# wing02/MyLdpcCppApi

Hardware: AMD Instinct MI355X
Metric: decoded Mbit/s (info bits), DVB-S2 N=64800 rate-1/2, 50 iters (higher is better)
Workload: dtype f32; 1 GPU; DVB-S2-profile (64800,32400) rate-1/2 (seeded IRA table with the standard's structure, E=226799), batch 4096 frames per GPU, 50 iterations, sum-product fp32 (probability domain), all-zero codeword + AWGN sigma=0.95 (no frame converges), early termination on, inputs resident in HBM; global_batch=4096, frames_per_gpu=4096, algo=sp, frames_per_launch=4096, parallelism=frames sharded over 1 GPU(s), all-gather of decoded bytes, frames_converged=0

## Files before the change

### myldpccppapi_amd/capi.py

```python
import ctypes

import numpy as np

from . import _lib
from ._lib import DecoderConfig, DecodeStats, LdpcError

ALGO_SP, ALGO_MS, ALGO_LAYERED, ALGO_MS_FUSED, ALGO_LAYERED_HOST = 0, 1, 2, 3, 4
MSG_F32, MSG_F16 = 0, 1
PACK_BYTES, PACK_BITS = 0, 1
CODE_PACKED, CODE_BITS = 0, 1
CODE_FORMATS = {"packed": CODE_PACKED, "bits": CODE_BITS}
PARITY_KINDS = {1: "dual_diagonal", 2: "staircase"}
HOST_INPUT = {"auto": 0, "staged": 1, "lock_pages": 2}
ALGOS = {"sp": ALGO_SP, "ms": ALGO_MS, "layered": ALGO_LAYERED, "ms_fused": ALGO_MS_FUSED,
         "layered_host": ALGO_LAYERED_HOST}

TUNE_FIELDS = {"fused": 0, "ldsp": 2, "ldsp_ext": 4, "ldsp_pack": 6, "link_narrow": 8, "check_wide": 10,
               "syn_xcd": 12, "fused_pack": 14, "fused_loop": 16, "device_tail": 18, "merge": 20, "link_deep": 22, "link_half": 24,
               "link_guided": 26, "tiles_first": 28}
TUNE_INTS = ("rows_per_wave", "cols_per_wave", "link_rows", "compact", "ldsp_grid", "ldsp_per_cu", "ldsp_waves", "place", "q_order")


def apply_tune(cfg, tune):
    flags, shape = 0, 0
    for k, v in (tune or {}).items():
        if k in TUNE_FIELDS:
            if v is not None:
                flags |= (1 if v else 2) << TUNE_FIELDS[k]
        elif k == "ldsp_per_cu":
            shape |= int(v) & 255
        elif k == "ldsp_waves":
            shape |= (int(v) & 255) << 8
        elif k in TUNE_INTS:
            setattr(cfg, "tune_" + k, int(v))
        else:
            raise KeyError("unknown tuning field %r" % k)
    cfg.tune_flags, cfg.tune_ldsp_shape = flags, shape


def hbm_probe(device=0, nbytes=1 << 30, reps=5, by_policy=False):
    g = ctypes.c_double(0.0)
    two = (ctypes.c_double * 2)(0.0, 0.0)
    _lib.check(_lib.load().ldpc_hbm_probe_device(int(device), int(nbytes), int(reps), ctypes.byref(g), two))
    return (g.value, two[0], two[1]) if by_policy else g.value


def hbm_sustained(device=0, nbytes=1 << 30, milliseconds=300):
    g = ctypes.c_double(0.0)
    _lib.check(_lib.load().ldpc_hbm_sustained_device(int(device), int(nbytes), int(milliseconds), ctypes.byref(g)))
    return g.value


def tune_from_env(env=None):
    import os
    env = os.environ if env is None else env
    t = {}
    for name, key in (("FUSED", "fused"), ("LDSP", "ldsp"), ("LDSP_EXT", "ldsp_ext"), ("LDSP_PACK", "ldsp_pack"),
                      ("LINK_NARROW", "link_narrow"), ("CHECK_WIDE", "check_wide"), ("SYN_XCD", "syn_xcd"),
                      ("FUSED_LOOP", "fused_loop"), ("DEVICE_TAIL", "device_tail"), ("MERGE", "merge"), ("LINK_DEEP", "link_deep"), ("LINK_HALF", "link_half"),
                      ("LINK_GUIDED", "link_guided"), ("TILES_FIRST", "tiles_first")):
        if "LDPC_TUNE_" + name in env:
            t[key] = int(env["LDPC_TUNE_" + name]) != 0
    if "LDPC_TUNE_NO_PACK" in env:
        t["fused_pack"] = False
    for name, key in (("RPW", "rows_per_wave"), ("CPW", "cols_per_wave"), ("LDSP_GRID", "ldsp_grid"),
                      ("LDSP_PER_CU", "ldsp_per_cu"), ("LDSP_WAVES", "ldsp_waves")):
        if "LDPC_TUNE_" + name in env:
            t[key] = int(env["LDPC_TUNE_" + name])
    for name, key in (("LINK_RPW", "link_rows"), ("COMPACT", "compact")):
# ... 275 lines not shown
```

### myldpccppapi_amd/csrc/flood_kernels.hpp

```cpp
#pragma once

#include <hip/hip_runtime.h>
#include <stdint.h>

#include "ldpc_expf.h"

namespace ldpc {

constexpr int kAlgoSP = 0;
constexpr int kAlgoMS = 1;
constexpr int kAlgoMSC = 2;
constexpr int kCompactCapacity = 512;
constexpr int kLastCapacity = 64;
constexpr int kBlock = 256;
constexpr int kWavesPerBlock = 4;
constexpr int kMaxUnrolledDegree = 16;
constexpr int kMaxUnrolledCheckDegreeMS = 32;

#ifndef LDPC_NT_LOAD
#define LDPC_NT_LOAD 1
#endif
#ifndef LDPC_NT_STORE
#define LDPC_NT_STORE 1
#endif
// ... 508 lines not shown
    const int32_t *__restrict__ extra_deg;
    int32_t n_extra;
    int32_t link_blocks;
    int32_t n_big, small_rows;
};

__host__ __device__ inline void link_chunk_rows(int c, int rows_per_wave, int n_big, int small_rows, int n_rows,
                                               int *rb, int *re)
{
    int b, e;
    if (c < n_big) { b = c * rows_per_wave; e = b + rows_per_wave; }
    else { b = n_big * rows_per_wave + (c - n_big) * small_rows; e = b + small_rows; }
    *rb = b < n_rows ? b : n_rows;
    *re = e < n_rows ? e : n_rows;
}
__host__ __device__ inline int link_chunk_count(int rows_per_wave, int n_big, int small_rows, int n_rows)
{
    const int rest = n_rows - n_big * rows_per_wave;
    return n_big + (rest > 0 ? (rest + small_rows - 1) / small_rows : 0);
}

template <int ALGO, int V, typename T>
__device__ __forceinline__ void link_extra_rows(const CheckArgs &a, const LinkArgs &g, int tile, int block)
{
    constexpr size_t F = 64 * V;
    const int lane = threadIdx.x & 63;
    const int w = (block - g.link_blocks) * kWavesPerBlock + wave_id_in_block();
    if (w >= g.n_extra) return;
    const T *Qu = static_cast<const T *>(a.Q) + (size_t)tile * (size_t)a.E * F;
    T *Rt = static_cast<T *>(a.R) + (size_t)tile * (size_t)a.E * F + (size_t)lane * V;
    check_row_generic<ALGO, V, T>(Qu, (unsigned)lane * V, Rt, g.extra_e0[w], g.extra_deg[w], a.qpos, ms_corr_of(a));
}

#ifdef LDPC_LINK_WIDE_WAVES
#define LDPC_LINK_WIDE_ATTR __attribute__((amdgpu_waves_per_eu(LDPC_LINK_WIDE_WAVES, LDPC_LINK_WIDE_WAVES)))
#else
#define LDPC_LINK_WIDE_ATTR
#endif
template <int ALGO, int D, int V, typename T>
__global__ __launch_bounds__(kBlock) LDPC_LINK_WIDE_ATTR void check_link_kernel(const CheckArgs a, const LinkArgs g)
{
    constexpr size_t F = 64 * V;
    const int lane = threadIdx.x & 63;
    const GridPos gp = grid_pos(a.tiles_first);
    const int tile = tile_select<V>(a.tail, a.done, gp.row);
    if (tile < 0) return;
    if (gp.block >= g.link_blocks) { link_extra_rows<ALGO, V, T>(a, g, tile, gp.block); return; }
    const int wave = gp.block * kWavesPerBlock + wave_id_in_block();
    int r_begin, r_end;
    link_chunk_rows(wave, a.rows_per_wave, g.n_big, g.small_rows, a.n_rows, &r_begin, &r_end);
    const size_t lane_off = (size_t)lane * V;
    const unsigned lane_q = (unsigned)lane * V;
    const T *Qt = static_cast<const T *>(a.Q) + (size_t)tile * (size_t)a.E * F;
    T *Qwt = static_cast<T *>(g.Qw) + (size_t)tile * (size_t)a.E * F;
    T *Rt = static_cast<T *>(a.R) + (size_t)tile * (size_t)a.E * F + lane_off;
    const T *chan_t = static_cast<const T *>(g.chan) + (size_t)tile * (size_t)g.N * F + lane_off;
    uint64_t *hard_t = g.hard + (size_t)tile * (size_t)g.N * V;
    uint64_t frozen[V];
#pragma unroll
    for (int v = 0; v < V; ++v) frozen[v] = a.done[(size_t)tile * V + v];

    int pend_col = -1, pend_edge = 0, pend_kb = 0;
    float pend_r[V];
#pragma unroll
    for (int v = 0; v < V; ++v) pend_r[v] = 0.0f;

    float x[D][V];
    int qc[D], qn[D];
#pragma unroll
    for (int k = 0; k < D; ++k) qc[k] = qn[k] = 0;
    if (r_begin < r_end) {
        row_slots<D>(a.qpos, a.cls_e0[r_begin], lane, qc);
#pragma unroll
        for (int k = 0; k < D; ++k) vload<V>(x[k], Qt + (size_t)qc[k] * F + lane_q);
    }
    for (int r = r_begin; r < r_end; ++r) {
        const int e0 = a.cls_e0[r];
        const int next_col = (r + 1 < r_end) ? g.link_col[r] : -1;
        const int pos = g.link_pos[r];
        const int ka = next_col >= 0 ? (pos & 255) : -1;
        const int kb = pend_col >= 0 ? pend_kb : -1;
        if (r + 1 < r_end) row_slots<D>(a.qpos, a.cls_e0[r + 1], lane, qn);
        float ch[V];
        uint64_t old_w[V];
        if (pend_col >= 0) {
            vload<V>(ch, chan_t + (size_t)pend_col * F);
#pragma unroll
            for (int v = 0; v < V; ++v) old_w[v] = hard_t[(size_t)pend_col * V + v];
        }
        float out[D][V];
        if (ALGO == kAlgoSP) check_sp<D, V>(x, out); else if (ALGO == kAlgoMS) check_ms<D, V>(x, out); else check_ms<D, V, true, T>(x, out, ms_corr_of(a));
        if (r + 1 < r_end) {
#pragma unroll
            for (int k = 0; k < D; ++k) vload<V>(x[k], Qt + (size_t)qn[k] * F + lane_q);
        }
#pragma unroll
        for (int k = 0; k < D; ++k)
            if ((k != ka && k != kb) || g.store_all) vstore<V>(Rt + (size_t)(e0 + k) * F, out[k]);

        if (pend_col >= 0) {
            float rr[2][V], q[2][V];
#pragma unroll
            for (int v = 0; v < V; ++v) {
                rr[0][v] = pend_r[v];
                float t = out[0][v];
#pragma unroll
                for (int k = 1; k < D; ++k) t = (k == kb) ? out[k][v] : t;
                rr[1][v] = t;
            }
            uint64_t new_w[V];
            if (ALGO == kAlgoSP) {
                float f0[V], f1[V];
                var_sp<2, V>(ch, rr, q, f0, f1);
#pragma unroll
                for (int v = 0; v < V; ++v) {
                    const bool oldb = (old_w[v] >> lane) & 1ull;
                    const bool b = (f0[v] > f1[v]) ? false : ((f0[v] < f1[v]) ? true : oldb);
                    new_w[v] = __ballot(b);
                }
            } else {
#pragma unroll
                for (int v = 0; v < V; ++v) {
                    float p = ch[v];
                    p += rr[0][v];
                    p += rr[1][v];
                    q[0][v] = p - rr[0][v];
                    q[1][v] = p - rr[1][v];
                    new_w[v] = __ballot(!(p > 0.0f));
                }
            }
            if (lane == 0) {
#pragma unroll
                for (int v = 0; v < V; ++v)
                    hard_t[(size_t)pend_col * V + v] = (old_w[v] & frozen[v]) | (new_w[v] & ~frozen[v]);
            }
            if (g.write_q) {
                int qw1 = qc[0];
#pragma unroll
                for (int k = 1; k < D; ++k) qw1 = (k == kb) ? qc[k] : qw1;
                vstore<V>(Qwt + (size_t)pend_edge * F + lane_q, q[0]);
                vstore<V>(Qwt + (size_t)qw1 * F + lane_q, q[1]);
            }
        }
        pend_col = next_col;
        if (next_col >= 0) {
            pend_edge = qc[0];
#pragma unroll
            for (int k = 1; k < D; ++k) pend_edge = (k == ka) ? qc[k] : pend_edge;
            pend_kb = (pos >> 8) & 255;
#pragma unroll
            for (int v = 0; v < V; ++v) {
                float t = out[0][v];
#pragma unroll
                for (int k = 1; k < D; ++k) t = (k == ka) ? out[k][v] : t;
                pend_r[v] = t;
            }
        }
#pragma unroll
        for (int k = 0; k < D; ++k) qc[k] = qn[k];
    }
}

template <int V> __device__ __forceinline__ uint64_t compress_stride(uint64_t x)
{
    if (V == 1) return x;
    if (V == 2) {
        x &= 0x5555555555555555ull;
        x = (x | (x >> 1)) & 0x3333333333333333ull;
        x = (x | (x >> 2)) & 0x0f0f0f0f0f0f0f0full;
        x = (x | (x >> 4)) & 0x00ff00ff00ff00ffull;
        x = (x | (x >> 8)) & 0x0000ffff0000ffffull;
        x = (x | (x >> 16)) & 0x00000000ffffffffull;
        return x;
    }
    x &= 0x1111111111111111ull;
    x = (x | (x >> 3)) & 0x0303030303030303ull;
    x = (x | (x >> 6)) & 0x000f000f000f000full;
    x = (x | (x >> 12)) & 0x000000ff000000ffull;
    x = (x | (x >> 24)) & 0x000000000000ffffull;
    return x;
}

template <int ALGO, int D, int V, typename T, int W = 1>
__global__ __launch_bounds__(kBlock) void check_link_narrow_kernel(const CheckArgs a, const LinkArgs g)
{
    constexpr size_t F = 64 * V;
    constexpr int SUBS = V / W;
    constexpr int FB = 64 / SUBS;
    const int lane = threadIdx.x & 63;
    const GridPos gp = grid_pos(a.tiles_first);
    const int tile = tile_select<V>(a.tail, a.done, gp.row);
    if (tile < 0) return;
// ... 1053 lines not shown
```

### myldpccppapi_amd/csrc/ldpc_hip.hip

```cpp
#include <hip/hip_runtime.h>

#include <algorithm>
#include <chrono>
#include <cstdarg>
#include <cstdio>
#include <cstdlib>
#include <cstring>
#include <map>
#include <memory>
#include <new>
#include <string>
#include <thread>
#include <vector>

#include "../../include/ldpc_hip.h"
#include "flood_kernels.hpp"
#include "flood_tables.hpp"
#include "layered_kernels.hpp"
#include "fused_kernels.hpp"
#include "ldsp_kernels.hpp"
#include "engines.hpp"
#include "channel_kernels.hpp"
#include "tune.hpp"
#include "host_stage.hpp"
// ... 138 lines not shown
    DevBuf<int32_t> row_ptr, edge_col, col_ptr, col_edge;
    DevBuf<int32_t> qpos, col_qedge;
    std::vector<int32_t> h_qpos;
    DevBuf<uint8_t> chan, Q, R;
    int msg_size = 4;
    InitFn init_fn = nullptr;
    DevBuf<uint64_t> hard, failw, done;
    DevBuf<int32_t> iters, active;
    std::vector<RowClass> row_classes;
    std::vector<ColClass> col_classes;
    std::vector<ClassGroup> check_groups, var_groups;
    std::vector<int> check_solo, var_solo;
    CheckGroupFn check_group_fn[kCheckBuckets] = {};
    int check_group_width = 1;
    VarGroupFn var_group_fn[kVarBuckets] = {};
    DevBuf<int32_t> extra_e0, extra_deg;
    int n_extra = 0;
    int64_t extra_edges = 0;
    CheckFn check_fn[ldpc::kMaxUnrolledCheckDegreeMS + 1] = {};
    CheckFn check_fn_wide[ldpc::kMaxUnrolledCheckDegreeMS + 1] = {};
    int max_check_unrolled = ldpc::kMaxUnrolledDegree;
    LinkFn link_fn[ldpc::kMaxUnrolledDegree + 1] = {};
    LinkFn link_narrow_fn[ldpc::kMaxUnrolledDegree + 1] = {};
    LinkFn link_deep_fn[ldpc::kMaxUnrolledDegree + 1] = {};
    LinkFn link_half_fn[ldpc::kMaxUnrolledDegree + 1] = {};
    int tune_link_deep = 0;
    ldpc::Tune tune;
    int tune_link_narrow = 1;
    bool link_calibrated = false;
    float link_cal_ms[3] = {0, 0, 0};
    int place_candidates = 0, place_kept = 0;
    float place_ms[16] = {};
    int link_rpw = 16;
    int tune_link_guided = 0;
    int tune_tiles_first = 0;
    int cus = 256;
    VarFn var_fn[ldpc::kMaxUnrolledDegree + 1] = {};

    ldpc::LayeredPlan layered;
    ldpc::FusedPlan fused;
    bool use_fused = false;
    ldpc::LdspPlan ldsp;
    bool use_ldsp = false;
    bool ms_corr = false;
    float ms_scale = 1.0f, ms_offset = 0.0f;

    hipStream_t stream = nullptr, copy_stream = nullptr;
    struct HostSlot {
        DevBuf<float> llr;
        DevBuf<uint8_t> out;
        DevBuf<int32_t> iters;
        uint8_t *h_out = nullptr;
        int32_t *h_iters = nullptr;
        uint8_t *h_head = nullptr;
        hipEvent_t h2d_done = nullptr, all_done = nullptr;
        bool busy = false;
        int64_t off = 0, n = 0, dst = 0, copy_bytes = 0;
        int32_t *h_sum = nullptr;
        int g_iterations = 0, g_tiles = 0, g_children = 0, g_child_f[3] = {0, 0, 0};
    } slot[3];
    struct CallCounts { bool valid = false; int32_t iterations = 0, batch_time = 0; int64_t frames = 0, converged = 0, frame_rounds = 0; } call;
    bool suppress_poll = false;
    int32_t *h_active = nullptr;
    struct RingChunk { uint8_t *h = nullptr; hipEvent_t ev = nullptr; bool used = false; };
    std::vector<RingChunk> ring;
    size_t ring_next = 0;
// ... 407 lines not shown
        }
    }
    d->last_iterations = launched;
    d->last_tiles = tiles;
    if (resume) return LDPC_OK;

    HIP_TRY(span_begin(d, s, 3));
    if (use_tail) tail_scatter_kernel<V><<<2048, kBlock, 0, s>>>(ta);
    {
        PackArgs pa{d->hard.p, out_dev, d->iters.p, iters_dev, frames, out_bytes, d->N, d->cfg.K,
                    d->cfg.pack_mode};
        if (d->cfg.pack_mode == LDPC_PACK_BYTES) {
            if (out_dev && frames) pack_kernel<V><<<pack_grid<V>(d->cfg.K, tiles), kBlock, 0, s>>>(pa);
        } else {
            const int64_t n = std::max<int64_t>(out_bytes, frames);
            dim3 grid((unsigned)((n + kBlock - 1) / kBlock));
            if (out_dev && frames) pack_kernel<V><<<grid, kBlock, 0, s>>>(pa);
        }
        summary_kernel<V><<<(unsigned)((frames + 255) / 256), 256, 0, s>>>(
            d->iters.p, d->done.p, d->failw.p, frames, 1, d->summary.p);
        if (!d->is_child && d->cfg.poll_interval == 0 && freeze && !d->summary_pending) {
            HIP_TRY(hipMemcpyAsync(d->h_summary, d->summary.p, 2 * sizeof(int32_t), hipMemcpyDeviceToHost, s));
            HIP_TRY(hipEventRecord(d->ev_summary, s));
            d->summary_pending = true;
        }
    }
    HIP_TRY(span_end(d, s));
    HIP_TRY(hipGetLastError());
    return LDPC_OK;
}

int build_classes(ldpc_decoder *d, const ldpc_graph *g)
{
    std::map<int, std::vector<int32_t>> rows_by_deg, cols_by_deg, rowids_by_deg;
    for (int32_t m = 0; m < g->M; ++m) {
        const int deg = g->row_ptr[m + 1] - g->row_ptr[m];
        if (deg > 0) { rows_by_deg[deg].push_back(g->row_ptr[m]); rowids_by_deg[deg].push_back(m); }
    }
    std::vector<char> fused_col((size_t)g->N, 0);
    d->row_classes.resize(rows_by_deg.size());
    size_t i = 0;
    for (auto &kv : rows_by_deg) {
        RowClass &rc = d->row_classes[i++];
        rc.degree = kv.first;
        rc.count = (int)kv.second.size();
        rc.h_e0 = kv.second;
        HIP_TRY(rc.e0.upload(kv.second));
        const std::vector<int32_t> &ids = rowids_by_deg[kv.first];
        const int rpw = d->link_rpw;
        if (rpw >= 2 && rc.degree >= 2 && rc.degree <= ldpc::kMaxUnrolledDegree) {
            rc.n_big = (rc.count + rpw - 1) / rpw;
            rc.small_rows = rpw;
            const int small = std::max(2, rpw / 4);
            const bool forced = ldpc::tune_forced_on(d->tune_link_guided);
            if ((d->T >= 4 || forced) && small < rpw && !ldpc::tune_forced_off(d->tune_link_guided)) {
                const int64_t last_generation = (int64_t)d->cus * 16 / d->T;
                int64_t big = (int64_t)rc.n_big - last_generation;
                if (big <= 0 && forced) big = rc.n_big - std::max(1, rc.n_big / 3);
                if (big > 0) { rc.n_big = (int)big; rc.small_rows = small; }
            }
            std::vector<char> chunk_end((size_t)rc.count, 0);
            for (int c = 0, nc = ldpc::link_chunk_count(rpw, rc.n_big, rc.small_rows, rc.count); c < nc; ++c) {
                int rb, re;
                ldpc::link_chunk_rows(c, rpw, rc.n_big, rc.small_rows, rc.count, &rb, &re);
                if (re > rb) chunk_end[(size_t)re - 1] = 1;
            }
            std::vector<int32_t> lcol((size_t)rc.count, -1), lpos((size_t)rc.count, 0);
            for (int idx = 0; idx + 1 < rc.count; ++idx) {
                if (chunk_end[idx]) continue;
                const int32_t m = ids[idx], m2 = ids[idx + 1];
                for (int32_t p = g->row_ptr[m]; p < g->row_ptr[m + 1]; ++p) {
                    const int32_t c = g->cols[p];
                    if (g->col_ptr[c + 1] - g->col_ptr[c] != 2 || fused_col[c]) continue;
                    const int32_t ea = g->col_edge[g->col_ptr[c]], eb = g->col_edge[g->col_ptr[c] + 1];
                    if (ea != p || g->rows[eb] != m2) continue;
                    lcol[idx] = c;
                    lpos[idx] = (p - g->row_ptr[m]) | ((eb - g->row_ptr[m2]) << 8);
                    fused_col[c] = 1;
                    ++rc.linked;
                    break;
                }
            }
            if (rc.linked * 4 >= rc.count) {
                HIP_TRY(rc.link_col.upload(lcol));
                HIP_TRY(rc.link_pos.upload(lpos));
            } else {
                for (int idx = 0; idx < rc.count; ++idx)
                    if (lcol[idx] >= 0) fused_col[lcol[idx]] = 0;
                rc.linked = 0;
            }
        }
    }
    for (int32_t n = 0; n < g->N; ++n) {
        const int deg = g->col_ptr[n + 1] - g->col_ptr[n];
        if (!fused_col[n]) cols_by_deg[deg].push_back(n);
    }
    d->col_classes.resize(cols_by_deg.size());
    i = 0;
    for (auto &kv : cols_by_deg) {
        ColClass &cc = d->col_classes[i++];
        cc.degree = kv.first;
        cc.count = (int)kv.second.size();
        std::vector<int32_t> edges;
        edges.reserve((size_t)cc.count * std::max(cc.degree, 1));
        for (int32_t n : kv.second)
            for (int32_t p = g->col_ptr[n]; p < g->col_ptr[n + 1]; ++p) edges.push_back(g->col_edge[p]);
        if (edges.empty()) edges.push_back(0);
        HIP_TRY(cc.col.upload(kv.second));
        HIP_TRY(cc.edge.upload(edges));
    }
    {
        d->h_qpos.assign((size_t)g->E, -1);
        int64_t slot = 0;
        if (d->tune.q_order >= 0)
            for (ColClass &cc : d->col_classes) {
                cc.q_base = slot;
                const std::vector<int32_t> &members = cols_by_deg[cc.degree];
                for (size_t ci = 0; ci < members.size(); ++ci)
                    for (int k = 0; k < cc.degree; ++k)
                        d->h_qpos[(size_t)g->col_edge[(size_t)g->col_ptr[members[ci]] + k]] = (int32_t)(slot + (int64_t)k * cc.count + (int64_t)ci);
                slot += (int64_t)cc.degree * cc.count;
            }
        for (int64_t e = 0; e < g->E; ++e)
            if (d->h_qpos[(size_t)e] < 0) d->h_qpos[(size_t)e] = d->tune.q_order >= 0 ? (int32_t)slot++ : (int32_t)e;
        std::vector<int32_t> cq((size_t)g->E);
        for (int64_t p = 0; p < g->E; ++p) cq[(size_t)p] = d->h_qpos[(size_t)g->col_edge[(size_t)p]];
        HIP_TRY(d->qpos.upload(d->h_qpos));
        HIP_TRY(d->col_qedge.upload(cq));
    }
    return LDPC_OK;
}

int plan_launches(ldpc_decoder *d)
{
    using ldpc::GroupClass;
    const int V = d->V;
    const bool merge = ldpc::tune_pick(d->tune.merge, true) && !d->tune_check_wide;
    d->check_groups.clear(); d->var_groups.clear(); d->check_solo.clear(); d->var_solo.clear();
    d->n_extra = 0; d->extra_edges = 0;
    int linked_classes = 0;
    int64_t unlinked_rows = 0;
    for (auto &rc : d->row_classes) { if (rc.linked) ++linked_classes; else unlinked_rows += rc.count; }
    const bool as_extra = merge && linked_classes == 1 && unlinked_rows > 0 && unlinked_rows <= 64;
    std::vector<int> cb[kCheckBuckets], vb[kVarBuckets];
    std::vector<int32_t> xe0, xdeg;
    for (int i = 0; i < (int)d->row_classes.size(); ++i) {
        RowClass &rc = d->row_classes[i];
        if (rc.linked) continue;
        if (as_extra) {
            for (int32_t e : rc.h_e0) { xe0.push_back(e); xdeg.push_back(rc.degree); d->extra_edges += rc.degree; }
            continue;
        }
        int b = -1;
        for (int k = 0; k < kCheckBuckets; ++k)
            if (rc.degree >= kCheckBucketLo[k] && rc.degree <= kCheckBucketHi[k] && rc.degree <= d->max_check_unrolled &&
                d->check_group_fn[k]) b = k;
        if (merge && b >= 0) cb[b].push_back(i); else d->check_solo.push_back(i);
    }
    if (as_extra) {
        d->n_extra = (int)xe0.size();
        HIP_TRY(d->extra_e0.upload(xe0));
        HIP_TRY(d->extra_deg.upload(xdeg));
    }
// ... 41 lines not shown
    return LDPC_OK;
}

int setup_flooding(ldpc_decoder *d, const ldpc_graph *g, size_t TF)
{
    const ldpc_decoder_config *cfg = &d->cfg;
    d->msg_size = cfg->msg_dtype == LDPC_MSG_F16 ? 2 : 4;
    HIP_TRY(d->chan.alloc(TF * d->N * d->msg_size));
    HIP_TRY(d->Q.alloc(TF * (size_t)d->E * d->msg_size));
    HIP_TRY(d->R.alloc(TF * (size_t)d->E * d->msg_size));
    int rc = build_classes(d, g);
    if (rc) return rc;
    ldpc::FloodFns fns;
    if (cfg->algo == LDPC_ALGO_SP) ldpc::fill_flood_sp(d->V, &fns);
    else if (d->ms_corr && cfg->msg_dtype == LDPC_MSG_F16) ldpc::fill_flood_msc16(d->V, &fns);
    else if (d->ms_corr) ldpc::fill_flood_msc(d->V, &fns);
    else if (cfg->msg_dtype == LDPC_MSG_F16) ldpc::fill_flood_ms16(d->V, &fns);
    else ldpc::fill_flood_ms(d->V, &fns);
    memcpy(d->check_fn, fns.check, sizeof fns.check);
    memcpy(d->check_fn_wide, fns.check_wide, sizeof fns.check_wide);
    memcpy(d->link_fn, fns.link, sizeof fns.link);
    memcpy(d->link_narrow_fn, fns.link_narrow, sizeof fns.link_narrow);
    memcpy(d->link_deep_fn, fns.link_deep, sizeof fns.link_deep);
    memcpy(d->link_half_fn, fns.link_half, sizeof fns.link_half);
    memcpy(d->var_fn, fns.var, sizeof fns.var);
    memcpy(d->check_group_fn, fns.check_group, sizeof fns.check_group);
    d->check_group_width = fns.check_group_width;
    memcpy(d->var_group_fn, fns.var_group, sizeof fns.var_group);
    d->init_fn = fns.init;
    d->max_check_unrolled = fns.max_check_unrolled;
    return plan_launches(d);
}

template <int V> int calibrate_link(ldpc_decoder *d)
{
    using namespace ldpc;
    RowClass *rcp = nullptr;
    for (auto &rc : d->row_classes) if (rc.linked) rcp = &rc;
    if (!rcp || !d->link_fn[rcp->degree] || !d->link_narrow_fn[rcp->degree]) return LDPC_OK;
    RowClass &rc = *rcp;
    const int tiles = d->T;
    hipStream_t s = d->stream;
    HIP_TRY(hipMemsetAsync(d->Q.p, 0, d->Q.n, s));
    HIP_TRY(hipMemsetAsync(d->chan.p, 0, d->chan.n, s));
    HIP_TRY(hipMemsetAsync(d->done.p, 0, d->done.n * sizeof(uint64_t), s));
    hipEvent_t ev[2] = {nullptr, nullptr};
    HIP_TRY(hipEventCreate(&ev[0]));
    HIP_TRY(hipEventCreate(&ev[1]));
    float best[3] = {1e30f, 1e30f, 1e30f};
    const int candidates = d->link_half_fn[rc.degree] ? 3 : 2;
    hipError_t err = hipSuccess;
    for (int rep = 0; rep < 4 && err == hipSuccess; ++rep) {
        for (int nar = 0; nar < candidates && err == hipSuccess; ++nar) {
            CheckArgs a{d->Q.p, d->R.p, rc.e0.p, d->done.p, d->E, rc.count, d->link_rpw, rc.degree, d->ms_scale,
                        TailRef{nullptr, 0, 0}};
            a.ms_offset = d->ms_offset;
            a.qpos = d->qpos.p;
            LinkArgs lk{rc.link_col.p, rc.link_pos.p, d->chan.p, d->Q.p, d->hard.p, d->N, 1, 0, nullptr, nullptr, 0, 0,
                        rc.n_big, rc.small_rows};
            const int waves = link_chunk_count(d->link_rpw, rc.n_big, rc.small_rows, rc.count) * (nar == 1 ? V : nar == 2 ? V / 2 : 1);
            lk.link_blocks = (waves + kWavesPerBlock - 1) / kWavesPerBlock;
            const dim3 grid = flood_grid(d, lk.link_blocks, tiles, &a.tiles_first, true);
            err = hipEventRecord(ev[0], s);
            (nar == 2 ? d->link_half_fn : nar == 1 ? d->link_narrow_fn : d->link_fn)[rc.degree]<<<grid, kBlock, 0, s>>>(a, lk);
            if (err == hipSuccess) err = hipEventRecord(ev[1], s);
            if (err == hipSuccess) err = hipEventSynchronize(ev[1]);
            float ms = 0;
            if (err == hipSuccess) err = hipEventElapsedTime(&ms, ev[0], ev[1]);
            if (err == hipSuccess && rep > 0 && ms < best[nar]) best[nar] = ms;
        }
    }
    (void)hipEventDestroy(ev[0]);
    (void)hipEventDestroy(ev[1]);
    if (err != hipSuccess) return fail(LDPC_ERR_HIP, "link calibration: %s", hipGetErrorString(err));
    HIP_TRY(hipGetLastError());
    int pick = 0;
    for (int k = 0; k < candidates; ++k) { d->link_cal_ms[k] = best[k]; if (best[k] < best[pick]) pick = k; }
    d->tune_link_narrow = pick;
    d->link_calibrated = true;
    return LDPC_OK;
}

template <int V> int time_check_phase(ldpc_decoder *d, float *ms_out)
{
    hipStream_t s = d->stream;
    HIP_TRY(hipMemsetAsync(d->Q.p, 0, d->Q.n, s));
    HIP_TRY(hipMemsetAsync(d->chan.p, 0, d->chan.n, s));
    HIP_TRY(hipMemsetAsync(d->done.p, 0, d->done.n * sizeof(uint64_t), s));
    hipEvent_t ev[2] = {nullptr, nullptr};
    HIP_TRY(hipEventCreate(&ev[0]));
    HIP_TRY(hipEventCreate(&ev[1]));
    float best = 1e30f;
    hipError_t err = hipSuccess;
    int rc = LDPC_OK;
    for (int rep = 0; rep < 4 && err == hipSuccess && rc == LDPC_OK; ++rep) {
        err = hipEventRecord(ev[0], s);
        rc = enqueue_check_phase<V>(d, s, d->T, (int64_t)d->T * d->F, 1, d->cfg.max_iter, false, ldpc::TailRef{nullptr, 0, 0});
        if (rc == LDPC_OK)
            rc = enqueue_var_phase<V>(d, s, d->T, (int64_t)d->T * d->F, 1, d->cfg.max_iter, false, ldpc::TailRef{nullptr, 0, 0});
        if (err == hipSuccess) err = hipEventRecord(ev[1], s);
        if (err == hipSuccess) err = hipEventSynchronize(ev[1]);
        float ms = 0;
        if (err == hipSuccess) err = hipEventElapsedTime(&ms, ev[0], ev[1]);
        if (err == hipSuccess && rep > 0 && ms < best) best = ms;
    }
    (void)hipEventDestroy(ev[0]);
    (void)hipEventDestroy(ev[1]);
    if (rc) return rc;
    if (err != hipSuccess) return fail(LDPC_ERR_HIP, "placement search: %s", hipGetErrorString(err));
    *ms_out = best;
    return LDPC_OK;
}
// ... 190 lines not shown
    if (cfg->frames_per_lane != 0 && cfg->frames_per_lane != 1 && cfg->frames_per_lane != 2 &&
        cfg->frames_per_lane != 4)
        return fail(LDPC_ERR_ARG, "frames_per_lane must be 0, 1, 2 or 4");
    if (cfg->msg_dtype != LDPC_MSG_F32 && cfg->msg_dtype != LDPC_MSG_F16)
        return fail(LDPC_ERR_ARG, "unknown msg_dtype %d", cfg->msg_dtype);
    if (cfg->msg_dtype == LDPC_MSG_F16 && cfg->algo != LDPC_ALGO_MS)
        return fail(LDPC_ERR_UNSUPPORTED, "fp16 messages are built for flooding min-sum only "
                    "(the probability-domain SP needs fp32 range; layered: not yet)");
    if (!ldpc::tune_valid(*cfg)) return fail(LDPC_ERR_ARG, "tuning / streams config fields out of range");

    int ndev = 0;
    HIP_TRY(hipGetDeviceCount(&ndev));
    if (cfg->device < 0 || cfg->device >= ndev)
        return fail(LDPC_ERR_HIP, "device %d not present (%d HIP devices)", cfg->device, ndev);
    HIP_TRY(hipSetDevice(cfg->device));

    ldpc_decoder *d = new (std::nothrow) ldpc_decoder;
    if (!d) return fail(LDPC_ERR_NOMEM, "out of memory");
    std::unique_ptr<ldpc_decoder> guard(d);
    d->cfg = *cfg;
    d->ms_corr = ms_corr;
    d->ms_scale = cfg->ms_scale != 0.0f ? cfg->ms_scale : 1.0f;
    d->ms_offset = cfg->ms_offset;
    d->M = g->M; d->N = g->N; d->E = g->E;
    d->h_col_ptr = g->col_ptr; d->h_col_edge = g->col_edge; d->h_rows = g->rows; d->h_cols = g->cols;
    const ldpc::Tune tune = d->tune = ldpc::tune_from_config(*cfg);
    d->tune_rpw = tune.rows_per_wave;
    d->tune_cpw = tune.cols_per_wave;
    d->tune_syn_xcd = ldpc::tune_pick(tune.syn_xcd, true);
    d->tune_check_wide = ldpc::tune_pick(tune.check_wide, false);
    d->tune_link_narrow = ldpc::tune_pick(tune.link_half, false) ? 2 : (ldpc::tune_pick(tune.link_narrow, true) ? 1 : 0);
    d->tune_link_deep = ldpc::tune_pick(tune.link_deep, false);
    if (tune.link_rows) d->link_rpw = tune.link_rows < 0 ? 0 : tune.link_rows;
    d->tune_link_guided = tune.link_guided;
    d->tune_tiles_first = tune.tiles_first;
    HIP_TRY(hipDeviceGetAttribute(&d->cus, hipDeviceAttributeMultiprocessorCount, cfg->device));
    d->V = pick_frames_per_lane(*cfg, g->max_row_deg, g->max_col_deg);
    d->F = 64 * d->V;
    d->T = (cfg->max_batch + d->F - 1) / d->F;
    if (d->T == 1 && !tune.link_rows) d->link_rpw = 4;

    HIP_TRY(hipStreamCreateWithFlags(&d->stream, hipStreamNonBlocking));
    HIP_TRY(hipEventCreate(&d->ev_begin));
    HIP_TRY(hipEventCreate(&d->ev_end));
    HIP_TRY(hipHostMalloc((void **)&d->h_active, sizeof(int32_t), hipHostMallocDefault));
    HIP_TRY(hipHostMalloc((void **)&d->h_summary, 2 * sizeof(int32_t), hipHostMallocDefault));
    HIP_TRY(hipEventCreateWithFlags(&d->ev_summary, hipEventDisableTiming));
    HIP_TRY(d->row_ptr.upload(g->row_ptr));
    HIP_TRY(d->edge_col.upload(g->cols));
    HIP_TRY(d->col_ptr.upload(g->col_ptr));
    HIP_TRY(d->col_edge.upload(g->col_edge));
    d->TO = (ldpc::kCompactCapacity + d->F - 1) / d->F;
    d->tail_enabled = cfg->early_term && cfg->poll_interval == 0 && ldpc::tune_pick(tune.device_tail, true) &&
                      (cfg->algo == LDPC_ALGO_SP || cfg->algo == LDPC_ALGO_MS) && d->T >= 4 * d->TO && t_child_depth == 0;
    if (!d->tail_enabled) d->TO = 0;
    d->TA = d->T + d->TO;
    const size_t TF = (size_t)d->TA * d->F;
    HIP_TRY(d->hard.alloc((size_t)d->TA * d->N * d->V));
    HIP_TRY(d->failw.alloc((size_t)(cfg->max_iter + 2) * d->TA * d->V));
    HIP_TRY(d->done.alloc((size_t)d->TA * d->V));
    HIP_TRY(d->iters.alloc(TF));
    HIP_TRY(d->active.alloc(1));
    HIP_TRY(d->summary.alloc(4));

    if (cfg->algo == LDPC_ALGO_MS_FUSED) {
        if (cfg->pack_mode != LDPC_PACK_BYTES && cfg->K % 8)
// ... 39 lines not shown
        d->layered.ms_offset = d->ms_offset;
        int rc = d->use_fused ? 0 : ldpc::layered_plan_create(&d->layered, g->M, g->N, g->E, g->row_ptr, g->cols,
                                                              cfg->layer_rows, d->T, d->V);
        if (rc == -1) return fail(LDPC_ERR_ARG, "layer_rows=%d must divide M=%d and rows of a layer "
                                  "must not share a column", cfg->layer_rows, g->M);
        if (rc) return fail(LDPC_ERR_HIP, "layered plan allocation failed: %s",
                            hipGetErrorString(hipGetLastError()));
    } else {
        if (d->ms_corr && ldpc::tune_forced_on(tune.fused) && ldpc::tune_forced_off(tune.ldsp))
            return fail(LDPC_ERR_UNSUPPORTED, "ms_scale / ms_offset: the LDS-resident flooding kernel (LDPC_TUNE_FUSED on, "
                        "LDPC_TUNE_LDSP off) carries no correction; the record or the streaming kernels do");
        if (cfg->msg_dtype == LDPC_MSG_F32 && cfg->layer_rows > 0 && cfg->frames_per_lane == 0 &&
            (cfg->pack_mode == LDPC_PACK_BYTES || cfg->K % 8 == 0)) {
            const bool small = (int64_t)cfg->max_batch * g->E <= (int64_t)1 << 23;
            if (!d->ms_corr && ldpc::tune_pick(tune.fused, small)) {
                HIP_TRY(ldpc::fused_plan_create(&d->fused, g->M, g->N, g->E, g->row_ptr, g->cols, cfg->layer_rows));
                d->use_fused = d->fused.eligible && (cfg->algo == LDPC_ALGO_MS || d->fused.eligible_sp);
            }
            if (cfg->algo == LDPC_ALGO_MS && !ldpc::tune_forced_off(tune.fused) && !ldpc::tune_forced_off(tune.ldsp)) {
                d->ldsp.corr = d->ms_corr;
                d->ldsp.mc = ldpc::MsCorr{d->ms_scale, d->ms_offset};
                HIP_TRY(ldpc::engine_ldsp_plan_create(&d->ldsp, g->M, g->N, g->E, g->row_ptr, g->cols, cfg->layer_rows,
                                               cfg->K, cfg->max_batch, cfg->device, tune, 1));
                if (d->ldsp.eligible && (ldpc::tune_forced_on(tune.ldsp) || d->ldsp.lds_bytes <= 80 * 1024))
                    d->use_fused = d->use_ldsp = true;
                else
                    ldpc::ldsp_plan_destroy(&d->ldsp);
            }
        }
        if (!d->use_fused) {
            int rc = setup_flooding(d, g, TF);
            if (rc) return rc;
            if (tune.link_narrow == 0 && tune.link_half == 0 && !tune.link_deep && d->V >= 2 && t_child_depth == 0) {
                rc = d->V == 1 ? calibrate_link<1>(d) : d->V == 2 ? calibrate_link<2>(d) : calibrate_link<4>(d);
                if (rc) return rc;
            }
            if (t_child_depth == 0) {
                rc = d->V == 1 ? placement_search<1>(d, TF) : d->V == 2 ? placement_search<2>(d, TF) : placement_search<4>(d, TF);
                if (rc) return rc;
            }
            if (d->tail_enabled) {
                HIP_TRY(d->tail_state.alloc(4));
                HIP_TRY(d->tail_map.alloc((size_t)d->TO * d->F));
                HIP_TRY(d->running.alloc((size_t)cfg->max_iter + 2));
            }
            if (t_child_depth == 0) d->child_capacity = cfg->max_batch >= 4096 ? 2 * ldpc::kCompactCapacity : ldpc::kCompactCapacity;
            else d->child_capacity = cfg->max_batch > ldpc::kCompactCapacity ? ldpc::kCompactCapacity : ldpc::kLastCapacity;
            d->compact_threshold = d->child_capacity;
            if (tune.compact) d->compact_threshold = tune.compact < 0 ? 0 : std::min(d->child_capacity, tune.compact);
            const bool may_have_child = t_child_depth == 0 || cfg->max_batch > ldpc::kLastCapacity;
            if (cfg->early_term && cfg->poll_interval > 0 && d->T > 1 && d->compact_threshold > 0 && may_have_child) {
                ldpc_decoder_config cc = *cfg;
                cc.max_batch = d->child_capacity;
                cc.frames_per_lane = (d->child_capacity > ldpc::kCompactCapacity && d->V == 4) ? 4 : 1;
                cc.layer_rows = 0;
                cc.tune_compact = d->child_capacity > ldpc::kLastCapacity ? 0 : -1;
                ++t_child_depth;
                rc = ldpc_decoder_create(g, &cc, &d->child);
                --t_child_depth;
                if (rc) return rc;
                d->child->is_child = true;
                HIP_TRY(hipSetDevice(cfg->device));
                HIP_TRY(d->cmap.alloc((size_t)d->child_capacity));
                HIP_TRY(d->cinv.alloc((size_t)d->T * d->F));
                HIP_TRY(d->cmoved.alloc((size_t)d->T * d->V));
            }
        }
// ... 889 lines not shown
```

### myldpccppapi_amd/csrc/tune.hpp

```cpp
#pragma once

#include "../../include/ldpc_hip.h"

namespace ldpc {

struct Tune {
    int fused = 0, ldsp = 0, ldsp_ext = 0, ldsp_pack = 0, link_narrow = 0, check_wide = 0, syn_xcd = 0,
        fused_pack = 0, fused_loop = 0, device_tail = 0, merge = 0, link_deep = 0, link_half = 0, link_guided = 0, tiles_first = 0;
    int rows_per_wave = 0, cols_per_wave = 0;
    int link_rows = 0;
    int compact = 0;
    int ldsp_grid = 0, ldsp_per_cu = 0, ldsp_waves = 0;
    int place = 0;
    int q_order = 0;
};

inline Tune tune_from_config(const ldpc_decoder_config &c)
{
    Tune t;
    auto f = [&](int field) { return (c.tune_flags >> field) & 3; };
    t.fused = f(LDPC_TUNE_FUSED);
    t.ldsp = f(LDPC_TUNE_LDSP);
    t.ldsp_ext = f(LDPC_TUNE_LDSP_EXT);
    t.ldsp_pack = f(LDPC_TUNE_LDSP_PACK);
    t.link_narrow = f(LDPC_TUNE_LINK_NARROW);
    t.check_wide = f(LDPC_TUNE_CHECK_WIDE);
    t.syn_xcd = f(LDPC_TUNE_SYN_XCD);
    t.fused_pack = f(LDPC_TUNE_FUSED_PACK);
    t.fused_loop = f(LDPC_TUNE_FUSED_LOOP);
    t.device_tail = f(LDPC_TUNE_DEVICE_TAIL);
    t.merge = f(LDPC_TUNE_MERGE);
    t.link_deep = f(LDPC_TUNE_LINK_DEEP);
    t.link_half = f(LDPC_TUNE_LINK_HALF);
    t.link_guided = f(LDPC_TUNE_LINK_GUIDED);
    t.tiles_first = f(LDPC_TUNE_TILES_FIRST);
    t.rows_per_wave = c.tune_rows_per_wave;
    t.cols_per_wave = c.tune_cols_per_wave;
    t.link_rows = c.tune_link_rows;
    t.compact = c.tune_compact;
    t.ldsp_grid = c.tune_ldsp_grid;
    t.ldsp_per_cu = c.tune_ldsp_shape & 255;
    t.ldsp_waves = (c.tune_ldsp_shape >> 8) & 255;
    t.place = c.tune_place;
    t.q_order = c.tune_q_order;
    return t;
}

inline bool tune_pick(int tri, bool dflt) { return tri == 1 ? true : (tri == 2 ? false : dflt); }
inline bool tune_forced_on(int tri) { return tri == 1; }
inline bool tune_forced_off(int tri) { return tri == 2; }

inline bool tune_valid(const ldpc_decoder_config &c)
{
    for (int field = 0; field <= LDPC_TUNE_TILES_FIRST; field += 2)
        if (((c.tune_flags >> field) & 3) == 3) return false;
    if (c.tune_flags >> (LDPC_TUNE_TILES_FIRST + 2)) return false;
    return c.tune_rows_per_wave >= 0 && c.tune_rows_per_wave <= 4096 && c.tune_cols_per_wave >= 0 &&
           c.tune_cols_per_wave <= 4096 && c.tune_link_rows >= -1 && c.tune_link_rows <= 4096 &&
           c.tune_compact >= -1 && c.tune_ldsp_grid >= 0 && c.tune_ldsp_shape >= 0 && c.tune_ldsp_shape < 65536 &&
           c.tune_place >= 0 && c.tune_place <= 8 && c.host_input >= 0 && c.host_input <= 2 && c.host_copy_threads >= 0 && c.host_copy_threads <= 16 &&
           c.tune_q_order >= -1 && c.tune_q_order <= 1;
}

}
```

Before: 1127 Mbit/s.

## Hand off linked-row boundary messages between waves through LDS in check-link kernel

```diff
diff --git a/myldpccppapi_amd/capi.py b/myldpccppapi_amd/capi.py
--- a/myldpccppapi_amd/capi.py
+++ b/myldpccppapi_amd/capi.py
@@ -18,13 +18,17 @@
 TUNE_FIELDS = {"fused": 0, "ldsp": 2, "ldsp_ext": 4, "ldsp_pack": 6, "link_narrow": 8, "check_wide": 10,
                "syn_xcd": 12, "fused_pack": 14, "fused_loop": 16, "device_tail": 18, "merge": 20, "link_deep": 22, "link_half": 24,
                "link_guided": 26, "tiles_first": 28}
+LINK_NO_BLOCK = 2048
 TUNE_INTS = ("rows_per_wave", "cols_per_wave", "link_rows", "compact", "ldsp_grid", "ldsp_per_cu", "ldsp_waves", "place", "q_order")
 
 
 def apply_tune(cfg, tune):
     flags, shape = 0, 0
+    no_block = False
     for k, v in (tune or {}).items():
-        if k in TUNE_FIELDS:
+        if k == "link_block":
+            no_block = v is not None and not v
+        elif k in TUNE_FIELDS:
             if v is not None:
                 flags |= (1 if v else 2) << TUNE_FIELDS[k]
         elif k == "ldsp_per_cu":
@@ -35,6 +39,10 @@
             setattr(cfg, "tune_" + k, int(v))
         else:
             raise KeyError("unknown tuning field %r" % k)
+    if no_block and cfg.tune_link_rows >= 0:
+        if cfg.tune_link_rows >= LINK_NO_BLOCK:
+            raise ValueError("link_block=False needs link_rows in [0, %d)" % LINK_NO_BLOCK)
+        cfg.tune_link_rows += LINK_NO_BLOCK
     cfg.tune_flags, cfg.tune_ldsp_shape = flags, shape
 
 
diff --git a/myldpccppapi_amd/csrc/check_link_row.inc b/myldpccppapi_amd/csrc/check_link_row.inc
--- /dev/null
+++ b/myldpccppapi_amd/csrc/check_link_row.inc
@@ -0,0 +1,64 @@
+{
+    const int e0 = a.cls_e0[r];
+    const int next_col = (r + 1 < r_end || pick_up) ? g.link_col[r] : -1;
+    const int pos = g.link_pos[r];
+    const int ka = next_col >= 0 ? (pos & 255) : -1;
+    const int kb = LDPC_LINK_ROW_FIRST ? dep_kb : (pend_col >= 0 ? pend_kb : -1);
+    if (r + 1 < r_end) row_slots<D>(a.qpos, a.cls_e0[r + 1], lane, qn);
+    float ch[V];
+    uint64_t old_w[V];
+    if (!LDPC_LINK_ROW_FIRST && pend_col >= 0) {
+        vload<V>(ch, chan_t + (size_t)pend_col * F);
+#pragma unroll
+        for (int v = 0; v < V; ++v) old_w[v] = hard_t[(size_t)pend_col * V + v];
+    }
+    float out[D][V];
+    if (ALGO == kAlgoSP) check_sp<D, V>(x, out); else if (ALGO == kAlgoMS) check_ms<D, V>(x, out); else check_ms<D, V, true, T>(x, out, ms_corr_of(a));
+    if (r + 1 < r_end) {
+#pragma unroll
+        for (int k = 0; k < D; ++k) vload<V>(x[k], Qt + (size_t)qn[k] * F + lane_q);
+    }
+#pragma unroll
+    for (int k = 0; k < D; ++k)
+        if ((k != ka && k != kb) || g.store_all) vstore<V>(Rt + (size_t)(e0 + k) * F, out[k]);
+
+    if (kb >= 0) {
+        float rr[2][V];
+#pragma unroll
+        for (int v = 0; v < V; ++v) {
+            rr[0][v] = pend_r[v];
+            float t = out[0][v];
+#pragma unroll
+            for (int k = 1; k < D; ++k) t = (k == kb) ? out[k][v] : t;
+            rr[1][v] = t;
+        }
+        int qw1 = qc[0];
+#pragma unroll
+        for (int k = 1; k < D; ++k) qw1 = (k == kb) ? qc[k] : qw1;
+        if (LDPC_LINK_ROW_FIRST) {
+#pragma unroll
+            for (int v = 0; v < V; ++v) hand_r[wib][v][lane] = rr[1][v];
+            if (lane == 0) hand_slot[wib] = qw1;
+        } else {
+            link_var_node<ALGO, V, T>(ch, old_w, rr, frozen, hard_t + (size_t)pend_col * V, lane, g.write_q,
+                                      Qwt + (size_t)pend_edge * F + lane_q, Qwt + (size_t)qw1 * F + lane_q);
+        }
+    }
+    if (LDPC_LINK_ROW_FIRST) __syncthreads();
+    pend_col = next_col;
+    if (next_col >= 0) {
+        pend_edge = qc[0];
+#pragma unroll
+        for (int k = 1; k < D; ++k) pend_edge = (k == ka) ? qc[k] : pend_edge;
+        pend_kb = (pos >> 8) & 255;
+#pragma unroll
+        for (int v = 0; v < V; ++v) {
+            float t = out[0][v];
+#pragma unroll
+            for (int k = 1; k < D; ++k) t = (k == ka) ? out[k][v] : t;
+            pend_r[v] = t;
+        }
+    }
+#pragma unroll
+    for (int k = 0; k < D; ++k) qc[k] = qn[k];
+}
diff --git a/myldpccppapi_amd/csrc/flood_kernels.hpp b/myldpccppapi_amd/csrc/flood_kernels.hpp
--- a/myldpccppapi_amd/csrc/flood_kernels.hpp
+++ b/myldpccppapi_amd/csrc/flood_kernels.hpp
@@ -564,6 +564,43 @@
     check_row_generic<ALGO, V, T>(Qu, (unsigned)lane * V, Rt, g.extra_e0[w], g.extra_deg[w], a.qpos, ms_corr_of(a));
 }
 
+template <int ALGO, int V, typename T>
+__device__ __forceinline__ void link_var_node(const float (&ch)[V], const uint64_t (&old_w)[V], const float (&rr)[2][V],
+                                              const uint64_t (&frozen)[V], uint64_t *hard_w, int lane, int write_q,
+                                              T *q0, T *q1)
+{
+    float q[2][V];
+    uint64_t new_w[V];
+    if (ALGO == kAlgoSP) {
+        float f0[V], f1[V];
+        var_sp<2, V>(ch, rr, q, f0, f1);
+#pragma unroll
+        for (int v = 0; v < V; ++v) {
+            const bool oldb = (old_w[v] >> lane) & 1ull;
+            const bool b = (f0[v] > f1[v]) ? false : ((f0[v] < f1[v]) ? true : oldb);
+            new_w[v] = __ballot(b);
+        }
+    } else {
+#pragma unroll
+        for (int v = 0; v < V; ++v) {
+            float p = ch[v];
+            p += rr[0][v];
+            p += rr[1][v];
+            q[0][v] = p - rr[0][v];
+            q[1][v] = p - rr[1][v];
+            new_w[v] = __ballot(!(p > 0.0f));
+        }
+    }
+    if (lane == 0) {
+#pragma unroll
+        for (int v = 0; v < V; ++v) hard_w[v] = (old_w[v] & frozen[v]) | (new_w[v] & ~frozen[v]);
+    }
+    if (write_q) {
+        vstore<V>(q0, q[0]);
+        vstore<V>(q1, q[1]);
+    }
+}
+
 #ifdef LDPC_LINK_WIDE_WAVES
 #define LDPC_LINK_WIDE_ATTR __attribute__((amdgpu_waves_per_eu(LDPC_LINK_WIDE_WAVES, LDPC_LINK_WIDE_WAVES)))
 #else
@@ -578,9 +615,15 @@
     const int tile = tile_select<V>(a.tail, a.done, gp.row);
     if (tile < 0) return;
     if (gp.block >= g.link_blocks) { link_extra_rows<ALGO, V, T>(a, g, tile, gp.block); return; }
-    const int wave = gp.block * kWavesPerBlock + wave_id_in_block();
+    const int wib = wave_id_in_block();
+    const int wave = gp.block * kWavesPerBlock + wib;
     int r_begin, r_end;
     link_chunk_rows(wave, a.rows_per_wave, g.n_big, g.small_rows, a.n_rows, &r_begin, &r_end);
+    __shared__ float hand_r[kWavesPerBlock][V][64];
+    __shared__ int hand_slot[kWavesPerBlock];
+    const int dep_kb = (wib > 0 && r_begin < r_end && r_begin > 0 && g.link_col[r_begin - 1] >= 0)
+                           ? ((g.link_pos[r_begin - 1] >> 8) & 255) : -1;
+    const bool pick_up = wib + 1 < kWavesPerBlock;
     const size_t lane_off = (size_t)lane * V;
     const unsigned lane_q = (unsigned)lane * V;
     const T *Qt = static_cast<const T *>(a.Q) + (size_t)tile * (size_t)a.E * F;
@@ -606,90 +649,32 @@
 #pragma unroll
         for (int k = 0; k < D; ++k) vload<V>(x[k], Qt + (size_t)qc[k] * F + lane_q);
     }
-    for (int r = r_begin; r < r_end; ++r) {
-        const int e0 = a.cls_e0[r];
-        const int next_col = (r + 1 < r_end) ? g.link_col[r] : -1;
-        const int pos = g.link_pos[r];
-        const int ka = next_col >= 0 ? (pos & 255) : -1;
-        const int kb = pend_col >= 0 ? pend_kb : -1;
-        if (r + 1 < r_end) row_slots<D>(a.qpos, a.cls_e0[r + 1], lane, qn);
-        float ch[V];
+    if (r_begin < r_end) {
+        const int r = r_begin;
+#define LDPC_LINK_ROW_FIRST 1
+#include "check_link_row.inc"
+#undef LDPC_LINK_ROW_FIRST
+    } else {
+        __syncthreads();
+    }
+    for (int r = r_begin + 1; r < r_end; ++r) {
+#define LDPC_LINK_ROW_FIRST 0
+#include "check_link_row.inc"
+#undef LDPC_LINK_ROW_FIRST
+    }
+    if (pend_col >= 0) {
+        float ch[V], rr[2][V];
         uint64_t old_w[V];
-        if (pend_col >= 0) {
-            vload<V>(ch, chan_t + (size_t)pend_col * F);
-#pragma unroll
-            for (int v = 0; v < V; ++v) old_w[v] = hard_t[(size_t)pend_col * V + v];
-        }
-        float out[D][V];
-        if (ALGO == kAlgoSP) check_sp<D, V>(x, out); else if (ALGO == kAlgoMS) check_ms<D, V>(x, out); else check_ms<D, V, true, T>(x, out, ms_corr_of(a));
-        if (r + 1 < r_end) {
-#pragma unroll
-            for (int k = 0; k < D; ++k) vload<V>(x[k], Qt + (size_t)qn[k] * F + lane_q);
-        }
-#pragma unroll
-        for (int k = 0; k < D; ++k)
-            if ((k != ka && k != kb) || g.store_all) vstore<V>(Rt + (size_t)(e0 + k) * F, out[k]);
-
-        if (pend_col >= 0) {
-            float rr[2][V], q[2][V];
-#pragma unroll
-            for (int v = 0; v < V; ++v) {
-                rr[0][v] = pend_r[v];
-                float t = out[0][v];
-#pragma unroll
-                for (int k = 1; k < D; ++k) t = (k == kb) ? out[k][v] : t;
-                rr[1][v] = t;
-            }
-            uint64_t new_w[V];
-            if (ALGO == kAlgoSP) {
-                float f0[V], f1[V];
-                var_sp<2, V>(ch, rr, q, f0, f1);
-#pragma unroll
-                for (int v = 0; v < V; ++v) {
-                    const bool oldb = (old_w[v] >> lane) & 1ull;
-                    const bool b = (f0[v] > f1[v]) ? false : ((f0[v] < f1[v]) ? true : oldb);
-                    new_w[v] = __ballot(b);
-                }
-            } else {
-#pragma unroll
-                for (int v = 0; v < V; ++v) {
-                    float p = ch[v];
-                    p += rr[0][v];
-                    p += rr[1][v];
-                    q[0][v] = p - rr[0][v];
-                    q[1][v] = p - rr[1][v];
-                    new_w[v] = __ballot(!(p > 0.0f));
-                }
-            }
-            if (lane == 0) {
-#pragma unroll
-                for (int v = 0; v < V; ++v)
-                    hard_t[(size_t)pend_col * V + v] = (old_w[v] & frozen[v]) | (new_w[v] & ~frozen[v]);
-            }
-            if (g.write_q) {
-                int qw1 = qc[0];
-#pragma unroll
-                for (int k = 1; k < D; ++k) qw1 = (k == kb) ? qc[k] : qw1;
-                vstore<V>(Qwt + (size_t)pend_edge * F + lane_q, q[0]);
-                vstore<V>(Qwt + (size_t)qw1 * F + lane_q, q[1]);
-            }
-        }
-        pend_col = next_col;
-        if (next_col >= 0) {
-            pend_edge = qc[0];
-#pragma unroll
-            for (int k = 1; k < D; ++k) pend_edge = (k == ka) ? qc[k] : pend_edge;
-            pend_kb = (pos >> 8) & 255;
-#pragma unroll
-            for (int v = 0; v < V; ++v) {
-                float t = out[0][v];
-#pragma unroll
-                for (int k = 1; k < D; ++k) t = (k == ka) ? out[k][v] : t;
-                pend_r[v] = t;
-            }
-        }
-#pragma unroll
-        for (int k = 0; k < D; ++k) qc[k] = qn[k];
+        vload<V>(ch, chan_t + (size_t)pend_col * F);
+#pragma unroll
+        for (int v = 0; v < V; ++v) old_w[v] = hard_t[(size_t)pend_col * V + v];
+        int lane_h = lane;
+        asm volatile("" : "+v"(lane_h));
+#pragma unroll
+        for (int v = 0; v < V; ++v) { rr[0][v] = pend_r[v]; rr[1][v] = hand_r[wib + 1][v][lane_h]; }
+        const int qw1 = __builtin_amdgcn_readfirstlane(hand_slot[wib + 1]);
+        link_var_node<ALGO, V, T>(ch, old_w, rr, frozen, hard_t + (size_t)pend_col * V, lane, g.write_q,
+                                  Qwt + (size_t)pend_edge * F + lane_q, Qwt + (size_t)qw1 * F + lane_q);
     }
 }
 
diff --git a/myldpccppapi_amd/csrc/ldpc_hip.hip b/myldpccppapi_amd/csrc/ldpc_hip.hip
--- a/myldpccppapi_amd/csrc/ldpc_hip.hip
+++ b/myldpccppapi_amd/csrc/ldpc_hip.hip
@@ -194,6 +194,7 @@
     int place_candidates = 0, place_kept = 0;
     float place_ms[16] = {};
     int link_rpw = 16;
+    bool link_block = true;
     int tune_link_guided = 0;
     int tune_tiles_first = 0;
     int cus = 256;
@@ -667,6 +668,9 @@
 
 int build_classes(ldpc_decoder *d, const ldpc_graph *g)
 {
+    const bool handoff = d->link_block && d->tune_link_narrow == 0;
+    d->row_classes.clear();
+    d->col_classes.clear();
     std::map<int, std::vector<int32_t>> rows_by_deg, cols_by_deg, rowids_by_deg;
     for (int32_t m = 0; m < g->M; ++m) {
         const int deg = g->row_ptr[m + 1] - g->row_ptr[m];
@@ -698,7 +702,7 @@
             for (int c = 0, nc = ldpc::link_chunk_count(rpw, rc.n_big, rc.small_rows, rc.count); c < nc; ++c) {
                 int rb, re;
                 ldpc::link_chunk_rows(c, rpw, rc.n_big, rc.small_rows, rc.count, &rb, &re);
-                if (re > rb) chunk_end[(size_t)re - 1] = 1;
+                if (re > rb && !(handoff && c % ldpc::kWavesPerBlock != ldpc::kWavesPerBlock - 1)) chunk_end[(size_t)re - 1] = 1;
             }
             std::vector<int32_t> lcol((size_t)rc.count, -1), lpos((size_t)rc.count, 0);
             for (int idx = 0; idx + 1 < rc.count; ++idx) {
@@ -764,6 +768,33 @@
         HIP_TRY(d->col_qedge.upload(cq));
     }
     return LDPC_OK;
+}
+
+struct FloodPlan {
+    std::vector<RowClass> row_classes;
+    std::vector<ColClass> col_classes;
+    DevBuf<int32_t> qpos, col_qedge, extra_e0, extra_deg;
+    std::vector<int32_t> h_qpos;
+    std::vector<ClassGroup> check_groups, var_groups;
+    std::vector<int> check_solo, var_solo;
+    int n_extra = 0;
+    int64_t extra_edges = 0;
+};
+static void plan_swap(ldpc_decoder *d, FloodPlan &p)
+{
+    std::swap(d->row_classes, p.row_classes);
+    std::swap(d->col_classes, p.col_classes);
+    std::swap(d->qpos, p.qpos);
+    std::swap(d->col_qedge, p.col_qedge);
+    std::swap(d->extra_e0, p.extra_e0);
+    std::swap(d->extra_deg, p.extra_deg);
+    std::swap(d->h_qpos, p.h_qpos);
+    std::swap(d->check_groups, p.check_groups);
+    std::swap(d->var_groups, p.var_groups);
+    std::swap(d->check_solo, p.check_solo);
+    std::swap(d->var_solo, p.var_solo);
+    std::swap(d->n_extra, p.n_extra);
+    std::swap(d->extra_edges, p.extra_edges);
 }
 
 int plan_launches(ldpc_decoder *d)
@@ -871,13 +902,31 @@
     return plan_launches(d);
 }
 
-template <int V> int calibrate_link(ldpc_decoder *d)
+template <int V> int calibrate_link(ldpc_decoder *d, const ldpc_graph *g)
 {
     using namespace ldpc;
     RowClass *rcp = nullptr;
     for (auto &rc : d->row_classes) if (rc.linked) rcp = &rc;
     if (!rcp || !d->link_fn[rcp->degree] || !d->link_narrow_fn[rcp->degree]) return LDPC_OK;
-    RowClass &rc = *rcp;
+    FloodPlan wide;
+    RowClass *rcw = rcp;
+    const int32_t *qpos_w = d->qpos.p;
+    if (d->link_block) {
+        const int form = d->tune_link_narrow;
+        FloodPlan mine;
+        plan_swap(d, mine);
+        d->tune_link_narrow = 0;
+        int rc = build_classes(d, g);
+        if (rc == LDPC_OK) rc = plan_launches(d);
+        d->tune_link_narrow = form;
+        plan_swap(d, wide);
+        plan_swap(d, mine);
+        if (rc) return rc;
+        rcw = nullptr;
+        for (auto &rc2 : wide.row_classes) if (rc2.linked) rcw = &rc2;
+        if (!rcw || rcw->degree != rcp->degree) return fail(LDPC_ERR_STATE, "link calibration: the two fusion plans disagree");
+        qpos_w = wide.qpos.p;
+    }
     const int tiles = d->T;
     hipStream_t s = d->stream;
     HIP_TRY(hipMemsetAsync(d->Q.p, 0, d->Q.n, s));
@@ -887,14 +936,15 @@
     HIP_TRY(hipEventCreate(&ev[0]));
     HIP_TRY(hipEventCreate(&ev[1]));
     float best[3] = {1e30f, 1e30f, 1e30f};
-    const int candidates = d->link_half_fn[rc.degree] ? 3 : 2;
+    const int candidates = d->link_half_fn[rcp->degree] ? 3 : 2;
     hipError_t err = hipSuccess;
     for (int rep = 0; rep < 4 && err == hipSuccess; ++rep) {
         for (int nar = 0; nar < candidates && err == hipSuccess; ++nar) {
+            RowClass &rc = nar == 0 ? *rcw : *rcp;
             CheckArgs a{d->Q.p, d->R.p, rc.e0.p, d->done.p, d->E, rc.count, d->link_rpw, rc.degree, d->ms_scale,
                         TailRef{nullptr, 0, 0}};
             a.ms_offset = d->ms_offset;
-            a.qpos = d->qpos.p;
+            a.qpos = nar == 0 ? qpos_w : d->qpos.p;
             LinkArgs lk{rc.link_col.p, rc.link_pos.p, d->chan.p, d->Q.p, d->hard.p, d->N, 1, 0, nullptr, nullptr, 0, 0,
                         rc.n_big, rc.small_rows};
             const int waves = link_chunk_count(d->link_rpw, rc.n_big, rc.small_rows, rc.count) * (nar == 1 ? V : nar == 2 ? V / 2 : 1);
@@ -917,6 +967,7 @@
     for (int k = 0; k < candidates; ++k) { d->link_cal_ms[k] = best[k]; if (best[k] < best[pick]) pick = k; }
     d->tune_link_narrow = pick;
     d->link_calibrated = true;
+    if (pick == 0 && d->link_block) plan_swap(d, wide);
     return LDPC_OK;
 }
 
@@ -1173,6 +1224,7 @@
     d->tune_link_narrow = ldpc::tune_pick(tune.link_half, false) ? 2 : (ldpc::tune_pick(tune.link_narrow, true) ? 1 : 0);
     d->tune_link_deep = ldpc::tune_pick(tune.link_deep, false);
     if (tune.link_rows) d->link_rpw = tune.link_rows < 0 ? 0 : tune.link_rows;
+    d->link_block = tune.link_block;
     d->tune_link_guided = tune.link_guided;
     d->tune_tiles_first = tune.tiles_first;
     HIP_TRY(hipDeviceGetAttribute(&d->cus, hipDeviceAttributeMultiprocessorCount, cfg->device));
@@ -1278,7 +1330,7 @@
             int rc = setup_flooding(d, g, TF);
             if (rc) return rc;
             if (tune.link_narrow == 0 && tune.link_half == 0 && !tune.link_deep && d->V >= 2 && t_child_depth == 0) {
-                rc = d->V == 1 ? calibrate_link<1>(d) : d->V == 2 ? calibrate_link<2>(d) : calibrate_link<4>(d);
+                rc = d->V == 1 ? calibrate_link<1>(d, g) : d->V == 2 ? calibrate_link<2>(d, g) : calibrate_link<4>(d, g);
                 if (rc) return rc;
             }
             if (t_child_depth == 0) {
diff --git a/myldpccppapi_amd/csrc/tune.hpp b/myldpccppapi_amd/csrc/tune.hpp
--- a/myldpccppapi_amd/csrc/tune.hpp
+++ b/myldpccppapi_amd/csrc/tune.hpp
@@ -9,11 +9,14 @@
         fused_pack = 0, fused_loop = 0, device_tail = 0, merge = 0, link_deep = 0, link_half = 0, link_guided = 0, tiles_first = 0;
     int rows_per_wave = 0, cols_per_wave = 0;
     int link_rows = 0;
+    bool link_block = true;
     int compact = 0;
     int ldsp_grid = 0, ldsp_per_cu = 0, ldsp_waves = 0;
     int place = 0;
     int q_order = 0;
 };
+
+constexpr int kTuneLinkNoBlock = 2048;
 
 inline Tune tune_from_config(const ldpc_decoder_config &c)
 {
@@ -37,6 +40,10 @@
     t.rows_per_wave = c.tune_rows_per_wave;
     t.cols_per_wave = c.tune_cols_per_wave;
     t.link_rows = c.tune_link_rows;
+    if (t.link_rows >= kTuneLinkNoBlock && t.link_rows < 2 * kTuneLinkNoBlock) {
+        t.link_block = false;
+        t.link_rows -= kTuneLinkNoBlock;
+    }
     t.compact = c.tune_compact;
     t.ldsp_grid = c.tune_ldsp_grid;
     t.ldsp_per_cu = c.tune_ldsp_shape & 255;
```

Result: no change. 1136 Mbit/s, median of 6 (+0.8%).
